# blyssprivacy/sdk

Hardware: NVIDIA H100
Metric: PIR server queries/sec (Spiral process_query) (higher is better)
Workload: dtype u64

## Files before the change

### sdk_b200/csrc/api.cu

```cuda
#include "api_internal.hpp"
#include "ntt_tables.hpp"
#include "update_body.hpp"
#include "gadget.hpp"
#include <cstdio>
#include <cerrno>
#include <fcntl.h>
#include <unistd.h>
#include <algorithm>
#include <cmath>
#include <memory>
#include <cstring>
#include <condition_variable>
#include <chrono>
#include <deque>
#include <mutex>
#include <set>
#include <utility>
#include <vector>

using namespace b200pir;

namespace b200pir {
thread_local unsigned long long g_kernel_launches = 0;
thread_local std::string g_last_error;

int fail(const std::exception& e) {
  cudaGetLastError();
  g_last_error = e.what();
  const Error* pe = dynamic_cast<const Error*>(&e);
  return pe ? pe->code : B200PIR_E_CUDA;
}

void opt_in_smem_impl(const void* kernel, int bytes) {
  static std::mutex mu;
  static std::set<std::pair<const void*, int>> done;
  int dev = 0;
  B200_CUDA(cudaGetDevice(&dev));
  std::lock_guard<std::mutex> lk(mu);
  if (done.count({kernel, dev})) return;
  B200_CUDA(cudaFuncSetAttribute(kernel, cudaFuncAttributeMaxDynamicSharedMemorySize, bytes));
  done.insert({kernel, dev});
}
}

namespace {

using b200pir::tables::build_tables;
using b200pir::tables::invmod;
uint64_t log2_ceil_u64(uint64_t a) { return (uint64_t)std::ceil(std::log2((double)a)); }
using b200pir::bits_per;
using b200pir::live_digits;
const uint64_t kQ2Values[37] = {0, 0, 0, 0, 0, 0, 0, 0, 0, 0, 0, 0, 0, 0, 12289ULL, 12289ULL, 61441ULL, 65537ULL,
                                65537ULL, 520193ULL, 786433ULL, 786433ULL, 3604481ULL, 7340033ULL, 16515073ULL,
                                33292289ULL, 67043329ULL, 132120577ULL, 268369921ULL, 469762049ULL, 1073479681ULL,
                                2013265921ULL, 4293918721ULL, 8588886017ULL, 17175674881ULL, 34359214081ULL,
                                68718428161ULL};

enum Stage { ST_EXPAND = 0, ST_MUL, ST_FROMNTT, ST_FOLD, ST_PACK, ST_ENCODE, ST_QIMG , ST_COUNT };

}

struct b200pir_ctx {
  int device = 0;
  cudaStream_t stream = nullptr;
  bool own_stream = true;
  std::recursive_mutex mu;
  b200pir_params hp;
  int dim0, num_per, slices, trials, g, stop_round, num_packing;
  int bits_gsw, bits_conv, bits_left, bits_right;
  int live_gsw, live_conv, live_left, live_right;
  bool has_right;
  uint64_t q2, q1, setup_bytes, query_bytes, response_bytes;
  int q1_bits;
  DevParams dp;
  DevBuf<Twiddle> d_tw;
  DevBuf<Twiddle> d_tw4k;
  DevBuf<uint32_t> d_neg1;
  int mul_variant = 0, max_group = 16, profile = 0;
  int sparse_fold = 0;
  int db_format = -1;
  DevBuf<uint2> w_qf;
  DevBuf<uint8_t> w_qt;
  int sm_count = 0;
  size_t ws_queries = 0, ws_rows = 0;
  DevBuf<uint64_t> w_query;
  DevBuf<uint32_t> w_v;
  DevBuf<uint32_t> w_zflags;
  DevBuf<uint32_t> w_xr;
  DevBuf<uint4> w_qdev;
  DevBuf<uint32_t> w_vfold, w_vfold_neg;
  DevBuf<uint32_t> w_mult;
  DevBuf<uint32_t> w_cts;
  const uint32_t* folded = nullptr;
  size_t folded_stride = 0;
  DevBuf<uint64_t> w_packed;
  DevBuf<uint8_t> w_resp;
  static constexpr size_t kWriteStageBytes = (size_t)64 << 20;
  static constexpr size_t kWriteStageItems = 65536;
  DevBuf<uint8_t> w_wbytes;
  DevBuf<ItemWrite> w_witems;
  std::mutex export_mu;
  uint8_t* h_export[2] = {nullptr, nullptr};
  size_t h_export_bytes = 0;
  cudaEvent_t export_done[2] = {nullptr, nullptr};
  void ensure_export_staging(size_t bytes) {
    w_wbytes.ensure(std::max(kWriteStageBytes, bytes));
    if (!export_done[0])
      for (auto& e : export_done) B200_CUDA(cudaEventCreateWithFlags(&e, cudaEventDisableTiming | cudaEventBlockingSync));
    if (bytes <= h_export_bytes) return;
    release_export_pinned();
    const size_t n = std::max(kWriteStageBytes, bytes);
    for (auto& h : h_export) B200_CUDA(cudaHostAlloc(reinterpret_cast<void**>(&h), n, cudaHostAllocDefault));
    h_export_bytes = n;
  }
  void release_export_pinned() {
    for (auto& h : h_export) { if (h) cudaFreeHost(h); h = nullptr; }
    h_export_bytes = 0;
  }
  struct Pending {
    b200pir_db* db; b200pir_pp* pp; const uint64_t* query_ct; const uint8_t* query_bytes; uint8_t* out;
    int rc = 0; std::string err; bool done = false;
  };
  static constexpr size_t kCoalesceMax = 32;
  static constexpr size_t kPassQueries = 16;
  int coalesce = 1;
  int coalesce_window_us = 200;
  size_t last_batch = 0;
  std::chrono::steady_clock::time_point last_batch_end{};
  std::mutex qmu;
  std::condition_variable qcv;
  std::deque<Pending*> pending;
  bool leader_active = false;
  unsigned long long coalesced_batches = 0, coalesced_queries = 0;
  DevBuf<const uint32_t*> d_pptab;
  size_t pptab_cap = 0;
  std::vector<const uint32_t*> h_pptab;
  b200pir_pp* const* multi_pps = nullptr;
  PpTable pp_table(b200pir_pp* pp, size_t count);
  struct Span { int stage; cudaEvent_t a, b; };
  std::vector<Span> spans;
  std::vector<cudaEvent_t> event_pool;
  size_t event_next = 0;
  int mul_launches = 0;
  double last_ms[9] = {0, 0, 0, 0, 0, 0, 0, 0, 0};

  size_t v_words() const { return ((size_t)1 << g) * 4 * POLY; }
  size_t fold_words() const { return (size_t)hp.nu_2 * 2 * 2 * hp.t_gsw * 2 * POLY; }
  MulGeom geom(int rows) const { return MulGeom{dim0, rows, slices}; }

  cudaEvent_t get_event() {
    if (event_next == event_pool.size()) {
      cudaEvent_t e;
      B200_CUDA(cudaEventCreate(&e));
      event_pool.push_back(e);
    }
    return event_pool[event_next++];
  }
  struct Scope {
    b200pir_ctx* c; int stage; cudaEvent_t a = nullptr;
    Scope(b200pir_ctx* ctx, int st) : c(ctx), stage(st) {
      if (c->profile) { a = c->get_event(); cudaEventRecord(a, c->stream); }
    }
    ~Scope() {
      if (c->profile) { cudaEvent_t b = c->get_event(); cudaEventRecord(b, c->stream); c->spans.push_back({stage, a, b}); }
    }
  };
  void prof_reset() { if (profile == 2) return; spans.clear(); event_next = 0; mul_launches = 0; }
  void prof_collect() {
    if (!profile) return;
    B200_CUDA(cudaStreamSynchronize(stream));
    for (int i = 0; i < 9; i++) last_ms[i] = 0;
    for (auto& s : spans) {
      float ms = 0;
      cudaEventElapsedTime(&ms, s.a, s.b);
      last_ms[s.stage == ST_QIMG ? 8 : s.stage] += ms;
      last_ms[6] += ms;
    }
    last_ms[7] = mul_launches;
  }
  void ensure_workspace_lite(size_t queries, size_t rows) {
    w_mult.ensure(queries * slices * rows * 4 * POLY);
    w_cts.ensure(queries * slices * rows * 4 * POLY);
    w_packed.ensure(queries * hp.instances * (hp.n + 1) * hp.n * POLY);
  }
  void ensure_workspace(size_t queries, size_t rows) {
    if (queries <= ws_queries && rows <= ws_rows) return;
    queries = std::max(queries, ws_queries);
    rows = std::max(rows, ws_rows);
    w_query.ensure(queries * 2 * POLY);
    if (hp.expand_queries) w_v.ensure(queries * v_words());
    w_qdev.ensure(queries * (size_t)dim0 * POLY);
    w_vfold.ensure(queries * std::max<size_t>(fold_words(), 1));
    w_vfold_neg.ensure(queries * std::max<size_t>(fold_words(), 1));
    w_mult.ensure(queries * slices * rows * 4 * POLY);
    w_cts.ensure(queries * slices * rows * 4 * POLY);
    w_packed.ensure(queries * hp.instances * (hp.n + 1) * hp.n * POLY);
    w_resp.ensure(queries * response_bytes);
    ws_queries = queries;
    ws_rows = rows;
  }
};

struct b200pir_db {
  b200pir_ctx* ctx;
  Shard shard;
  int rows;
  DbLayout layout;
  DevBuf<uint8_t> store;
  bool zmajor_product() const { return layout.format != 0; }
  uint4* slice0_base(int s, DevBuf<uint8_t>& scratch) {
    if (layout.format == 0) return reinterpret_cast<uint4*>(store.p);
    const size_t slice0_bytes = imad_cell(layout.G, 1, 0, 0, 0) * sizeof(uint4);
    if (!scratch.p) scratch.alloc(slice0_bytes);
    return reinterpret_cast<uint4*>(reinterpret_cast<uintptr_t>(scratch.p) - (uintptr_t)s * slice0_bytes);
  }
  void place_slice0(int s, const DevBuf<uint8_t>& scratch, cudaStream_t st) {
    const uint4* src = reinterpret_cast<const uint4*>(scratch.p);
    if (layout.format == 1) launch_db_to_frag(layout.F, src, reinterpret_cast<uint4*>(store.p), s, st);
    else if (layout.format == 2) launch_db_to_tc5(layout.T, src, store.p, s, st);
  }
  std::vector<uint64_t> present;
  uint64_t present_count = 0;
  std::vector<uint32_t> h_tile_mask;
  DevBuf<uint32_t> tile_mask;
  uint64_t capacity() const { return (uint64_t)ctx->slices * rows * ctx->dim0; }
  void presence_init() {
    present.assign((capacity() + 63) / 64, 0);
    present_count = 0;
    h_tile_mask.assign((size_t)ctx->slices * layout.T.mt, 0u);
    tile_mask.alloc(h_tile_mask.size());
    B200_CUDA(cudaMemsetAsync(tile_mask.p, 0, h_tile_mask.size() * 4, ctx->stream));
  }
  bool mark_host(int slice, int il, int j) {
    const uint64_t bit = ((uint64_t)slice * rows + il) * ctx->dim0 + j;
    if (!((present[bit >> 6] >> (bit & 63)) & 1)) { present[bit >> 6] |= 1ull << (bit & 63); present_count++; }
    const size_t w = (size_t)slice * layout.T.mt + (il >> 5);
    const uint32_t nv = h_tile_mask[w] | (1u << (j >> 5));
    if (nv == h_tile_mask[w]) return false;
    h_tile_mask[w] = nv;
    return true;
  }
  void mark(int slice, int il, int j, cudaStream_t s) {
    if (mark_host(slice, il, j)) {
      const size_t w = (size_t)slice * layout.T.mt + (il >> 5);
      B200_CUDA(cudaMemcpyAsync(tile_mask.p + w, &h_tile_mask[w], 4, cudaMemcpyHostToDevice, s));
    }
  }
  void mark_items(const ItemWrite* items, size_t count, cudaStream_t s) {
    bool changed = false;
    for (size_t k = 0; k < count; k++)
      for (int sl = 0; sl < ctx->slices; sl++) changed |= mark_host(sl, (int)items[k].il, (int)items[k].j);
    if (changed)
      B200_CUDA(cudaMemcpyAsync(tile_mask.p, h_tile_mask.data(), h_tile_mask.size() * 4, cudaMemcpyHostToDevice, s));
  }
  void mark_slice(int slice, cudaStream_t s) {
    const uint64_t lo = (uint64_t)slice * rows * ctx->dim0, hi = lo + (uint64_t)rows * ctx->dim0;
    for (uint64_t b = lo; b < hi; b++)
      if (!((present[b >> 6] >> (b & 63)) & 1)) { present[b >> 6] |= 1ull << (b & 63); present_count++; }
    const Tc5Geom& T = layout.T;
    const uint32_t full = T.ks >= 32 ? 0xffffffffu : ((1u << T.ks) - 1u);
    for (int m = 0; m < T.mt; m++) h_tile_mask[(size_t)slice * T.mt + m] = full;
    B200_CUDA(cudaMemcpyAsync(tile_mask.p + (size_t)slice * T.mt, &h_tile_mask[(size_t)slice * T.mt], (size_t)T.mt * 4,
                              cudaMemcpyHostToDevice, s));
  }
};

struct b200pir_pp {
  b200pir_ctx* ctx;
  DevBuf<uint32_t> pack, left, right, conv;
};

PpTable b200pir_ctx::pp_table(b200pir_pp* pp, size_t count) {
  if (count > pptab_cap) {
    pptab_cap = std::max<size_t>(count, 16);
    d_pptab.alloc(4 * pptab_cap);
    h_pptab.clear();
  }
  std::vector<const uint32_t*> h(4 * pptab_cap, nullptr);
  for (size_t i = 0; i < count; i++) {
    const b200pir_pp* p = multi_pps ? multi_pps[i] : pp;
    h[0 * pptab_cap + i] = p->pack.p;
    h[1 * pptab_cap + i] = p->left.p;
    h[2 * pptab_cap + i] = p->right.p ? p->right.p : p->left.p;
    h[3 * pptab_cap + i] = p->conv.p;
  }
  if (h != h_pptab) {
    B200_CUDA(cudaMemcpyAsync(d_pptab.p, h.data(), h.size() * sizeof(const uint32_t*), cudaMemcpyHostToDevice, stream));
    h_pptab = h;
  }
  return PpTable{d_pptab.p, d_pptab.p + pptab_cap, d_pptab.p + 2 * pptab_cap, d_pptab.p + 3 * pptab_cap};
}

namespace {

struct Guard {
  std::lock_guard<std::recursive_mutex> lk;
  explicit Guard(b200pir_ctx* c) : lk(c->mu) { cudaSetDevice(c->device); }
};

void upload_narrow(b200pir_ctx* c, uint32_t* dst, DevBuf<uint64_t>& wide, const uint64_t* host, size_t words) {
  wide.ensure(words);
  B200_CUDA(cudaMemcpyAsync(wide.p, host, words * 8, cudaMemcpyHostToDevice, c->stream));
  launch_narrow(dst, wide.p, words, c->stream);
}
void download_widen(b200pir_ctx* c, uint64_t* host, const uint32_t* src, size_t words) {
  DevBuf<uint64_t> wide(words);
  launch_widen(wide.p, src, words, c->stream);
  B200_CUDA(cudaMemcpyAsync(host, wide.p, words * 8, cudaMemcpyDeviceToHost, c->stream));
  B200_CUDA(cudaStreamSynchronize(c->stream));
}
void upload_ntt32(b200pir_ctx* c, DevBuf<uint32_t>& dst, const uint64_t* host, size_t words) {
  dst.alloc(words);
  DevBuf<uint64_t> wide;
  upload_narrow(c, dst.p, wide, host, words);
  B200_CUDA(cudaStreamSynchronize(c->stream));
}


void run_coefficient_expansion(b200pir_ctx* c, b200pir_pp* pp, uint32_t* v, size_t v_stride, int nq, bool all_slots) {
  const auto& hp = c->hp;
  cudaStream_t s = c->stream;
  const int g = c->g;
  const int stop_round = hp.nu_2 > 0 ? c->stop_round : 0;
  const int max_right = hp.nu_2 > 0 ? (int)(hp.t_gsw * hp.nu_2) : 0;
  const PpTable T = c->pp_table(pp, (size_t)nq);
  for (int r = 0; r < g; r++) {
    const int num_in = 1 << r;
    ExpandRound R;
    R.r = r; R.num_in = num_in; R.stop_round = stop_round; R.max_bits_to_gen_right = max_right;
    R.fill_skipped = all_slots ? 1 : 0;
    R.t_auto = (POLY >> r) + 1;
    R.t_left = (int)hp.t_exp_left; R.bits_left = c->bits_left; R.live_left = c->live_left;
    R.tab_left = T.left; R.off_left = (size_t)r * 2 * hp.t_exp_left * 2 * POLY;
    if (hp.nu_2 > 0 && c->has_right) {
      int rr = r <= c->stop_round ? r : c->stop_round;
      R.t_right = (int)hp.t_exp_right; R.bits_right = c->bits_right; R.live_right = c->live_right;
      R.tab_right = T.right; R.off_right = (size_t)rr * 2 * hp.t_exp_right * 2 * POLY;
    } else {
      R.t_right = R.t_left; R.bits_right = R.bits_left; R.live_right = R.live_left; R.tab_right = T.left; R.off_right = R.off_left;
    }
    const size_t xr_stride = (size_t)num_in * 2 * POLY;
    c->w_xr.ensure((size_t)nq * xr_stride);
    launch_expand_round_res(c->dp, v, v_stride, c->w_xr.p, xr_stride, nq, R, c->d_neg1.p + (size_t)r * 2 * POLY, s);
  }
}

void run_expand_query(b200pir_ctx* c, b200pir_pp* pp, const uint64_t* query_raw, uint32_t* v, uint4* q_dev,
                      uint32_t* v_fold, int nq, uint8_t* images = nullptr) {
  const auto& hp = c->hp;
  cudaStream_t s = c->stream;
  launch_to_ntt_strided(c->dp, v, c->v_words(), query_raw, (size_t)2 * POLY, 2, nq, s);
  run_coefficient_expansion(c, pp, v, c->v_words(), nq, false);
  const int factor = hp.nu_2 > 0 ? 2 : 1;
  if (images) {
    const Tc5Geom T = make_tc5_geom(c->dim0, 32);
    for (int q0 = 0; q0 < nq; q0 += 16)
      launch_reorient_to_tc5(T, v + (size_t)q0 * c->v_words(), c->v_words(), factor, std::min(16, nq - q0),
                             images + (size_t)(q0 / 16) * tc5_query_bytes(T), s);
  } else {
    launch_reorient(c->geom(c->num_per), q_dev, (size_t)c->dim0 * POLY, v, c->v_words(), nq, factor, s);
  }
  if (hp.nu_2 > 0)
    launch_regev_to_gsw(c->dp, v_fold, c->fold_words(), v, c->v_words(), nq, (int)hp.nu_2, 2, 1, c->pp_table(pp, (size_t)nq).conv,
                        (int)hp.t_gsw, (int)hp.t_conv, c->bits_conv, c->live_conv, s);
}

void run_fold(b200pir_ctx* c, uint64_t* cts, size_t batch, size_t batch_stride, size_t num, int k0,
              const uint32_t* vfold, const uint32_t* vfold_neg, int slices_per_query) {
  const size_t mat = (size_t)2 * 2 * c->hp.t_gsw * 2 * POLY;
  int k = k0;
  for (size_t half = num / 2; half >= 1; half /= 2, k--) {
    launch_fold_round(c->dp, cts, batch, batch_stride, (int)half, vfold + (size_t)k * mat, vfold_neg + (size_t)k * mat,
                      c->fold_words(), slices_per_query, (int)c->hp.t_gsw, c->bits_gsw, c->stream);
  }
}

const uint32_t* run_fold_res(b200pir_ctx* c, uint32_t* a, uint32_t* b, size_t batch, size_t batch_stride, size_t num,
                             int k0, const uint32_t* vfold, int slices_per_query) {
  const size_t mat = (size_t)2 * 2 * c->hp.t_gsw * 2 * POLY;
  int k = k0;
  uint32_t* src = a;
  uint32_t* dst = b;
  uint32_t* zero_flags = nullptr;
  if (c->sparse_fold) {
    c->w_zflags.ensure(batch * num);
    zero_flags = c->w_zflags.p;
  }
  for (size_t half = num / 2; half >= 1; half /= 2, k--) {
    launch_fold_res(c->dp, src, dst, batch, batch_stride, (int)half, vfold + (size_t)k * mat, c->fold_words(),
                    slices_per_query, (int)c->hp.t_gsw, c->bits_gsw, c->live_gsw, zero_flags, c->stream);
    std::swap(src, dst);
  }
  return src;
}

void run_prepare(b200pir_ctx* c, b200pir_pp* pp, size_t count, bool images = false) {
  b200pir_ctx::Scope sc(c, ST_EXPAND);
  if (images) c->w_qt.ensure((count + 15) / 16 * tc5_query_bytes(make_tc5_geom(c->dim0, 32)));
  if (c->hp.expand_queries)
    run_expand_query(c, pp, c->w_query.p, c->w_v.p, c->w_qdev.p, c->w_vfold.p, (int)count, images ? c->w_qt.p : nullptr);
}

void run_first_dim(b200pir_ctx* c, b200pir_db* db, size_t count, const uint4* qdev, uint32_t* out, int slice_begin,
                   int slice_count, const uint8_t* images = nullptr, size_t per_group = 16) {
  const DbLayout& L = db->layout;
  const size_t q_stride = (size_t)c->dim0 * POLY;
  const size_t out_stride = (size_t)c->slices * db->rows * 4 * POLY;
  if (L.format == 0) {
    b200pir_ctx::Scope sc(c, ST_MUL);
    size_t qi = 0;
    while (qi < count) {
      int nq = 1;
      if (count - qi >= 4 && c->max_group >= 4) nq = 4;
      else if (count - qi >= 2 && c->max_group >= 2) nq = 2;
      launch_multiply(c->dp, L.G, reinterpret_cast<const uint4*>(L.base), qdev + qi * q_stride, out + qi * out_stride,
                      slice_begin, slice_count, nq, q_stride, out_stride, c->mul_variant, c->stream);
      c->mul_launches++;
      qi += nq;
    }
  } else if (L.format == 2) {
    if (!images) c->w_qt.ensure(tc5_query_bytes(L.T));
    const size_t step = images ? per_group : 16;
    for (size_t qi = 0, g = 0; qi < count; qi += step, g++) {
      const int nq = (int)std::min<size_t>(step, count - qi);
      const uint8_t* qt = images ? images + g * tc5_query_bytes(L.T) : c->w_qt.p;
      if (!images) {
        b200pir_ctx::Scope sq(c, ST_QIMG);
        launch_query_to_tc5(L.T, qdev + qi * q_stride, q_stride, nq, c->w_qt.p, c->stream);
      }
      b200pir_ctx::Scope sc(c, ST_MUL);
      launch_multiply_tc5(c->dp, L.T, L.base, db->tile_mask.p, qt, out + qi * out_stride, out_stride, nq, slice_begin,
                          slice_count, c->sm_count, c->stream);
      c->mul_launches++;
    }
  } else {
    c->w_qf.ensure(imma_query_cells(L.F));
    const size_t per_pass = (c->max_group >= 16 && imma_supports_16(L.F)) ? 16 : (c->max_group >= 8 ? 8 : 4);
    for (size_t qi = 0; qi < count; qi += per_pass) {
      const int nq = (int)std::min<size_t>(per_pass, count - qi);
      {
        b200pir_ctx::Scope sq(c, ST_QIMG);
        launch_query_to_frag(L.F, qdev + qi * q_stride, q_stride, nq, c->w_qf.p, c->stream);
      }
      {
        b200pir_ctx::Scope sc(c, ST_MUL);
        launch_multiply_imma(c->dp, L.F, reinterpret_cast<const uint4*>(L.base), c->w_qf.p, out + qi * out_stride, out_stride,
                             nq, slice_begin, slice_count, c->stream);
        c->mul_launches++;
      }
    }
  }
}

void run_first_dim_and_fold(b200pir_ctx* c, b200pir_db* db, size_t count, const uint4* qdev = nullptr,
                            const uint32_t* vfold = nullptr, const uint8_t* images = nullptr, size_t per_group = 16) {
  if (!qdev) qdev = c->w_qdev.p;
  if (!vfold) vfold = c->w_vfold.p;
  const int rows = db->rows;
  const size_t out_stride = (size_t)c->slices * rows * 4 * POLY;
  const bool zmajor = db->zmajor_product();
  run_first_dim(c, db, count, qdev, zmajor ? c->w_cts.p : c->w_mult.p, 0, c->slices, images, per_group);
  {
    b200pir_ctx::Scope sc(c, ST_FROMNTT);
    if (zmajor) launch_intt_from_zmajor(c->dp, db->layout.F, c->w_cts.p, out_stride, c->w_mult.p, (int)count, c->slices, c->stream);
    else launch_ntt32(c->dp, c->w_mult.p, count * c->slices * rows * 2, true, c->stream);
  }
  {
    b200pir_ctx::Scope sc(c, ST_FOLD);
    c->folded = c->w_mult.p;
    c->folded_stride = (size_t)rows * 4 * POLY;
    if (rows > 1)
      c->folded = run_fold_res(c, c->w_mult.p, c->w_cts.p, count * c->slices, (size_t)rows * 4 * POLY, rows,
                               (int)c->hp.nu_2 - 1, vfold, c->slices);
  }
}

void run_pack_encode(b200pir_ctx* c, b200pir_pp* pp, const uint32_t* folded, size_t ct_stride, size_t count,
                     uint8_t* out_dev) {
  const auto& hp = c->hp;
  const size_t packed_words = (size_t)hp.instances * (hp.n + 1) * hp.n * POLY;
  {
    b200pir_ctx::Scope sc(c, ST_PACK);
    launch_pack(c->dp, c->w_packed.p, packed_words, folded, ct_stride, (size_t)c->slices * ct_stride, (int)count, c->pp_table(pp, count).pack,
                (int)hp.n, (int)hp.instances, (int)hp.t_conv, c->bits_conv, c->live_conv, (int)hp.version, c->stream);
  }
  {
    b200pir_ctx::Scope sc(c, ST_ENCODE);
    launch_encode(c->dp, out_dev, c->response_bytes, c->w_packed.p, packed_words, (int)count, (int)hp.n, (int)hp.instances,
                  c->q2, (int)hp.q2_bits, c->q1, c->q1_bits, c->stream);
  }
}

bool same_params(const b200pir_ctx* a, const b200pir_ctx* b) {
  return a == b || (a->device == b->device && std::memcmp(&a->hp, &b->hp, sizeof(b200pir_params)) == 0);
}
void check_db(b200pir_ctx* c, b200pir_db* db) {
  if (!db || !same_params(db->ctx, c)) throw Error(B200PIR_E_BADARG, "db handle was created for different parameters / device");
}
void check_pp(b200pir_ctx* c, b200pir_pp* pp) {
  if (!pp || !same_params(pp->ctx, c)) throw Error(B200PIR_E_BADARG, "pp handle was created for different parameters / device");
}

}

extern "C" {

const char* b200pir_last_error(void) { return g_last_error.c_str(); }
int b200pir_device_count(void) {
  int n = 0;
  if (cudaGetDeviceCount(&n) != cudaSuccess) return 0;
  return n;
}

int b200pir_ctx_create(const b200pir_params* params, int device, b200pir_ctx** out) {
  API_BEGIN
  if (!params || !out) throw Error(B200PIR_E_BADARG, "null argument");
  use_device(device);
  std::unique_ptr<b200pir_ctx> c(new b200pir_ctx());
  c->device = device;
  B200_CUDA(cudaDeviceGetAttribute(&c->sm_count, cudaDevAttrMultiProcessorCount, device));
  c->hp = *params;
  auto& hp = c->hp;
  if (hp.q2_bits < 14) hp.q2_bits = 14;
  if (hp.q2_bits > 36) throw Error(B200PIR_E_BADARG, "q2_bits out of range");
  if (hp.instances == 0) hp.instances = 1;
  if (hp.n < 1 || hp.n > 4) throw Error(B200PIR_E_UNSUPPORTED, "n must be 1..4");
  if (hp.nu_1 < 1 || hp.nu_1 > 16 || hp.nu_2 > 16) throw Error(B200PIR_E_BADARG, "nu_1/nu_2 out of range");
  if (hp.version > 1) throw Error(B200PIR_E_BADARG, "unknown version");
  if (hp.p < 2 || (hp.p & (hp.p - 1)) || hp.p > (1u << 20)) throw Error(B200PIR_E_BADARG, "p must be a power of two <= 2^20");
  for (uint64_t t : {hp.t_gsw, hp.t_conv, hp.t_exp_left, hp.t_exp_right})
    if (t < 3 || t > 56)
      throw Error(B200PIR_E_UNSUPPORTED, "gadget dimensions must be in 3..56");
  if (hp.db_item_size == 0) hp.db_item_size = hp.instances * hp.n * hp.n * 2048 * log2_ceil_u64(hp.p) / 8;
  c->dim0 = 1 << hp.nu_1;
  c->num_per = 1 << hp.nu_2;
  c->trials = (int)(hp.n * hp.n);
  c->slices = (int)(hp.instances * c->trials);
  c->g = (int)log2_ceil_u64(hp.t_gsw * hp.nu_2 + c->dim0);
  c->stop_round = hp.nu_2 ? (int)log2_ceil_u64(hp.t_gsw * hp.nu_2) : 0;
  if (c->g > 11) throw Error(B200PIR_E_UNSUPPORTED, "expansion needs more than 2048 slots");
  if (hp.expand_queries && hp.nu_2 > 0 && 2 * std::max<uint64_t>(c->dim0, hp.t_gsw * hp.nu_2) > (1ull << c->g))
    throw Error(B200PIR_E_UNSUPPORTED, "expansion: dim0 and t_gsw * nu_2 must each fit in half of the 2^g slots");
  c->num_packing = hp.version == 0 ? (int)hp.n : 2;
  c->has_right = hp.expand_queries && (hp.version == 0 || hp.t_exp_right != hp.t_exp_left);
  c->bits_gsw = bits_per((int)hp.t_gsw);
  c->bits_conv = bits_per((int)hp.t_conv);
  c->bits_left = bits_per((int)hp.t_exp_left);
  c->bits_right = bits_per((int)hp.t_exp_right);
  c->live_gsw = live_digits((int)hp.t_gsw);
  c->live_conv = live_digits((int)hp.t_conv);
  c->live_left = live_digits((int)hp.t_exp_left);
  c->live_right = live_digits((int)hp.t_exp_right);
  c->q2 = kQ2Values[hp.q2_bits];
  c->q1 = 4 * hp.p;
  c->q1_bits = (int)log2_ceil_u64(c->q1);
  {
    uint64_t bits = hp.instances * (hp.q2_bits * hp.n * 2048 + (uint64_t)c->q1_bits * hp.n * hp.n * 2048);
    c->response_bytes = ((bits + 63) / 64) * 8;
    uint64_t sz = (uint64_t)c->num_packing * hp.n * hp.t_conv;
    if (hp.expand_queries) {
      uint64_t right = (uint64_t)(c->stop_round + 1) * hp.t_exp_right;
      if (hp.version > 0 && hp.t_exp_left == hp.t_exp_right) right = 0;
      sz += (uint64_t)c->g * hp.t_exp_left + right + 2 * hp.t_conv;
    }
    c->setup_bytes = 32 + sz * 2048 * 8;
    uint64_t qp = hp.expand_queries ? 1 : (uint64_t)c->dim0 + hp.nu_2 * 2 * hp.t_gsw;
    c->query_bytes = 32 + qp * 2048 * 8;
  }
  B200_CUDA(cudaStreamCreateWithFlags(&c->stream, cudaStreamNonBlocking));
  const uint64_t q0 = 268369921ULL, q1m = 249561089ULL;
  std::vector<Twiddle> f0, i0, f1, i1;
  build_tables(q0, f0, i0);
  build_tables(q1m, f1, i1);
  std::vector<Twiddle> l0, l1;
  b200pir::tables::build_inverse_table_lz(q0, l0);
  b200pir::tables::build_inverse_table_lz(q1m, l1);
  c->d_tw.alloc(6 * POLY);
  const size_t tw_bytes = POLY * sizeof(Twiddle);
  B200_CUDA(cudaMemcpyAsync(c->d_tw.p + 4 * POLY, l0.data(), tw_bytes, cudaMemcpyHostToDevice, c->stream));
  B200_CUDA(cudaMemcpyAsync(c->d_tw.p + 5 * POLY, l1.data(), tw_bytes, cudaMemcpyHostToDevice, c->stream));
  B200_CUDA(cudaMemcpyAsync(c->d_tw.p, f0.data(), tw_bytes, cudaMemcpyHostToDevice, c->stream));
  B200_CUDA(cudaMemcpyAsync(c->d_tw.p + POLY, i0.data(), tw_bytes, cudaMemcpyHostToDevice, c->stream));
  B200_CUDA(cudaMemcpyAsync(c->d_tw.p + 2 * POLY, f1.data(), tw_bytes, cudaMemcpyHostToDevice, c->stream));
  B200_CUDA(cudaMemcpyAsync(c->d_tw.p + 3 * POLY, i1.data(), tw_bytes, cudaMemcpyHostToDevice, c->stream));
  std::vector<Twiddle> lo(2 * 3 * 64);
  for (int i = 0; i < 64; i++) { lo[(0 * 3 + 0) * 64 + i] = f0[i]; lo[(0 * 3 + 1) * 64 + i] = i0[i]; lo[(0 * 3 + 2) * 64 + i] = l0[i];
                                 lo[(1 * 3 + 0) * 64 + i] = f1[i]; lo[(1 * 3 + 1) * 64 + i] = i1[i]; lo[(1 * 3 + 2) * 64 + i] = l1[i]; }
  upload_poly_constants(lo.data(), c->stream);
  upload_mul_constants(lo.data(), c->stream);
  upload_imma_constants(lo.data(), c->stream);
  std::vector<Twiddle> tw4k;
  for (const uint64_t q : {q0, q1m}) {
    std::vector<Twiddle> f, i;
    build_tables(q, f, i, 4096, 12);
    tw4k.insert(tw4k.end(), f.begin(), f.end());
    tw4k.insert(tw4k.end(), i.begin(), i.end());
  }
  c->d_tw4k.alloc(tw4k.size());
  B200_CUDA(cudaMemcpyAsync(c->d_tw4k.p, tw4k.data(), tw4k.size() * sizeof(Twiddle), cudaMemcpyHostToDevice, c->stream));
  DevParams& dp = c->dp;
  dp.q[0] = (uint32_t)q0; dp.q[1] = (uint32_t)q1m;
  dp.cr1[0] = (uint64_t)(((u128)1 << 64) / q0);
  dp.cr1[1] = (uint64_t)(((u128)1 << 64) / q1m);
  dp.modulus = q0 * q1m;
  dp.cr1_mod = (uint64_t)(((u128)1 << 64) / dp.modulus);
  dp.q1_inv_mod_q0 = (uint32_t)invmod(q1m % q0, q0);
  dp.fwd[0] = c->d_tw.p; dp.inv[0] = c->d_tw.p + POLY; dp.fwd[1] = c->d_tw.p + 2 * POLY; dp.inv[1] = c->d_tw.p + 3 * POLY;
  dp.inv_lz[0] = c->d_tw.p + 4 * POLY; dp.inv_lz[1] = c->d_tw.p + 5 * POLY;
  dp.mu58[0] = (uint32_t)(((uint64_t)1 << 58) / q0); dp.mu58[1] = (uint32_t)(((uint64_t)1 << 58) / q1m);
  {
    std::vector<uint32_t> h((size_t)NTT_LOG_N * 2 * POLY, 0);
    for (int i = 0; i < NTT_LOG_N; i++) {
      int idx = POLY - (1 << i);
      h[((size_t)i * 2 + 0) * POLY + idx] = (uint32_t)(q0 - 1);
      h[((size_t)i * 2 + 1) * POLY + idx] = (uint32_t)(q1m - 1);
    }
    c->d_neg1.alloc(h.size());
    B200_CUDA(cudaMemcpyAsync(c->d_neg1.p, h.data(), h.size() * 4, cudaMemcpyHostToDevice, c->stream));
    launch_ntt32(dp, c->d_neg1.p, NTT_LOG_N, false, c->stream);
    B200_CUDA(cudaStreamSynchronize(c->stream));
  }
  B200_CUDA(cudaGetLastError());
  *out = c.release();
  API_END
}

void b200pir_ctx_destroy(b200pir_ctx* c) {
  if (!c) return;
  cudaSetDevice(c->device);
  cudaDeviceSynchronize();
  for (auto e : c->event_pool) cudaEventDestroy(e);
  c->release_export_pinned();
  for (auto e : c->export_done) if (e) cudaEventDestroy(e);
  if (c->own_stream && c->stream) cudaStreamDestroy(c->stream);
  delete c;
}
int b200pir_ctx_set_stream(b200pir_ctx* c, void* cuda_stream) {
  API_BEGIN
  if (!c) throw Error(B200PIR_E_BADARG, "null ctx");
  Guard gd(c);
  B200_CUDA(cudaStreamSynchronize(c->stream));
  if (c->own_stream && c->stream) cudaStreamDestroy(c->stream);
  c->stream = (cudaStream_t)cuda_stream;
  c->own_stream = false;
  API_END
}
int b200pir_ctx_synchronize(b200pir_ctx* c) {
  API_BEGIN
  if (!c) throw Error(B200PIR_E_BADARG, "null ctx");
  Guard gd(c);
  B200_CUDA(cudaStreamSynchronize(c->stream));
  B200_CUDA(cudaGetLastError());
  API_END
}
int b200pir_ctx_reserve(b200pir_ctx* c, size_t queries, size_t rows_local) {
  API_BEGIN
  if (!c) throw Error(B200PIR_E_BADARG, "null ctx");
  if (queries == 0 || queries > 4096 || rows_local == 0 || rows_local > ((size_t)1 << c->hp.nu_2))
    throw Error(B200PIR_E_BADARG, "reserve: 1..4096 queries, 1..num_per rows");
  Guard gd(c);
  B200_CUDA(cudaStreamSynchronize(c->stream));
  c->ensure_workspace(queries, rows_local);
  B200_CUDA(cudaGetLastError());
  API_END
}
int b200pir_ctx_set_option(b200pir_ctx* c, const char* key, int64_t value) {
  API_BEGIN
  if (!c || !key) throw Error(B200PIR_E_BADARG, "null argument");
  Guard gd(c);
  std::string k(key);
  if (k == "mul_variant") c->mul_variant = (int)value;
  else if (k == "batch") { if (value != 1 && value != 2 && value != 4 && value != 8 && value != 16) throw Error(B200PIR_E_BADARG, "batch must be 1, 2, 4, 8 or 16"); c->max_group = (int)value; }
  else if (k == "fold_variant" || k == "intt_variant" || k == "imma_variant" || k == "expand_variant" ||
           k == "expand_pair_min_ctas") {}
  else if (k == "sparse_fold") c->sparse_fold = value != 0;
  else if (k == "coalesce") c->coalesce = value != 0;
  else if (k == "coalesce_window_us") { if (value < 0 || value > 100000) throw Error(B200PIR_E_BADARG, "coalesce_window_us must be 0..100000"); c->coalesce_window_us = (int)value; }
  else if (k == "db_format") { if (value < -1 || value > 2) throw Error(B200PIR_E_BADARG, "db_format must be -1 (automatic), 0, 1 or 2"); c->db_format = (int)value; }
  else if (k == "profile") {
    if (value < 0 || value > 2) throw Error(B200PIR_E_BADARG, "profile must be 0, 1 or 2");
    c->profile = (int)value;
    c->spans.clear(); c->event_next = 0; c->mul_launches = 0;
  }
  else throw Error(B200PIR_E_BADARG, "unknown option " + k);
  API_END
}
int b200pir_ctx_sizes(b200pir_ctx* c, uint64_t* setup_bytes, uint64_t* query_bytes, uint64_t* response_bytes) {
  API_BEGIN
  if (!c) throw Error(B200PIR_E_BADARG, "null ctx");
  if (setup_bytes) *setup_bytes = c->setup_bytes;
  if (query_bytes) *query_bytes = c->query_bytes;
  if (response_bytes) *response_bytes = c->response_bytes;
  API_END
}

int b200pir_db_create(b200pir_ctx* c, uint64_t shard_index, uint64_t shard_count, b200pir_db** out) {
  API_BEGIN
  if (!c || !out) throw Error(B200PIR_E_BADARG, "null argument");
  Guard gd(c);
  if (shard_count == 0) { shard_count = 1; shard_index = 0; }
  if (shard_index >= shard_count || (shard_count & (shard_count - 1)) || (uint64_t)c->num_per % shard_count)
    throw Error(B200PIR_E_BADARG, "shard_count must be a power of two dividing num_per");
  std::unique_ptr<b200pir_db> db(new b200pir_db());
  db->ctx = c;
  db->shard = Shard{(int)shard_index, (int)shard_count};
  db->rows = c->num_per / (int)shard_count;
  DbLayout& L = db->layout;
  L.G = c->geom(db->rows);
  L.F = make_imma_geom(c->dim0, db->rows);
  L.T = make_tc5_geom(c->dim0, db->rows);
  L.format = c->db_format >= 0 ? c->db_format : (tc5_supported(L.T) ? 2 : 1);
  db->presence_init();
  if (L.format == 2 && !tc5_supported(L.T)) throw Error(B200PIR_E_UNSUPPORTED, "db_format 2: dim0 too large for the wgmma kernel");
  db->store.alloc(db_bytes(L, c->slices));
  L.base = db->store.p;
  B200_CUDA(cudaMemsetAsync(db->store.p, 0, db->store.n, c->stream));
  B200_CUDA(cudaStreamSynchronize(c->stream));
  *out = db.release();
  API_END
}
void b200pir_db_destroy(b200pir_db* db) {
  if (!db) return;
  cudaSetDevice(db->ctx->device);
  delete db;
}
extern "C++" {
namespace {
template <typename Fetch>
void upload_slice_impl(b200pir_ctx* c, b200pir_db* db, uint64_t slice, Fetch fetch) {
  const size_t per_z = (size_t)c->dim0 * c->num_per;
  int zc = (int)std::max<size_t>(1, std::min<size_t>(POLY, ((size_t)64 << 20) / (per_z * 8)));
  DevBuf<uint64_t> stage(per_z * zc);
  const MulGeom& G = db->layout.G;
  DevBuf<uint8_t> scratch;
  uint4* dst = db->slice0_base((int)slice, scratch) + imad_cell(G, (int)slice, 0, 0, 0);
  for (int z0 = 0; z0 < POLY; z0 += zc) {
    int cur = std::min(zc, POLY - z0);
    const uint64_t* src = fetch((size_t)z0 * per_z, per_z * cur);
    B200_CUDA(cudaMemcpyAsync(stage.p, src, per_z * cur * 8, cudaMemcpyHostToDevice, c->stream));
    launch_db_retile_chunk(G, db->shard, dst, stage.p, z0, cur, c->stream);
    B200_CUDA(cudaStreamSynchronize(c->stream));
  }
  db->place_slice0((int)slice, scratch, c->stream);
  db->mark_slice((int)slice, c->stream);
  B200_CUDA(cudaStreamSynchronize(c->stream));
  B200_CUDA(cudaGetLastError());
}

void write_items(b200pir_ctx* c, b200pir_db* db, const uint8_t* host, size_t span, const ItemWrite* items, size_t count) {
  if (count == 0) return;
  c->w_wbytes.ensure(std::max(b200pir_ctx::kWriteStageBytes, span));
  c->w_witems.ensure(std::max(b200pir_ctx::kWriteStageItems, count));
  if (span) B200_CUDA(cudaMemcpyAsync(c->w_wbytes.p, host, span, cudaMemcpyHostToDevice, c->stream));
  B200_CUDA(cudaMemcpyAsync(c->w_witems.p, items, count * sizeof(ItemWrite), cudaMemcpyHostToDevice, c->stream));
  const size_t chunks = (size_t)c->slices;
  const size_t bpc = (c->hp.db_item_size + chunks - 1) / chunks;
  launch_write_items(c->dp, db->layout, c->w_wbytes.p, c->w_witems.p, (int)count, (int)chunks, (int)bpc, c->hp.p, c->stream);
}

template <typename Sink>
void export_impl(b200pir_ctx* c, b200pir_db* db, int slice_begin, int slice_end, Sink sink) {
  std::lock_guard<std::mutex> ex(c->export_mu);
  const size_t per_z = (size_t)db->rows * c->dim0;
  const int zc = (int)std::max<size_t>(1, std::min<size_t>(POLY, b200pir_ctx::kWriteStageBytes / (per_z * 8)));
  struct Chunk { int slice, z0, zc; };
  std::vector<Chunk> chunks;
  for (int s = slice_begin; s < slice_end; s++)
    for (int z0 = 0; z0 < POLY; z0 += zc) chunks.push_back(Chunk{s, z0, std::min(zc, POLY - z0)});
  {
    Guard gd(c);
    c->ensure_export_staging(per_z * zc * 8);
  }
  auto consume = [&](size_t k) {
    const int b = (int)(k & 1);
    B200_CUDA(cudaEventSynchronize(c->export_done[b]));
    sink(chunks[k].slice, chunks[k].z0, chunks[k].zc, reinterpret_cast<const uint64_t*>(c->h_export[b]));
  };
  try {
    for (size_t k = 0; k < chunks.size(); k++) {
      {
        Guard gd(c);
        uint64_t* stage = reinterpret_cast<uint64_t*>(c->w_wbytes.p);
        launch_db_export(db->layout, chunks[k].slice, chunks[k].z0, chunks[k].zc, stage, c->stream);
        B200_CUDA(cudaMemcpyAsync(c->h_export[k & 1], stage, per_z * chunks[k].zc * 8, cudaMemcpyDeviceToHost, c->stream));
        B200_CUDA(cudaEventRecord(c->export_done[k & 1], c->stream));
      }
      if (k > 0) consume(k - 1);
    }
    if (!chunks.empty()) consume(chunks.size() - 1);
  } catch (...) {
    for (auto e : c->export_done) cudaEventSynchronize(e);
    throw;
  }
  B200_CUDA(cudaGetLastError());
}

void download_impl(b200pir_ctx* c, b200pir_db* db, int slice_begin, int slice_end, uint64_t* words) {
  const size_t d0 = (size_t)c->dim0, npg = (size_t)c->num_per, rows = (size_t)db->rows;
  const size_t G = (size_t)db->shard.count, gi = (size_t)db->shard.index;
  const size_t slice_words = d0 * npg * POLY;
  export_impl(c, db, slice_begin, slice_end, [&](int s, int z0, int zc, const uint64_t* src) {
    uint64_t* dst = words + (size_t)(s - slice_begin) * slice_words + (size_t)z0 * npg * d0;
    if (G == 1) { std::memcpy(dst, src, (size_t)zc * rows * d0 * 8); return; }
    for (size_t zl = 0; zl < (size_t)zc; zl++)
      for (size_t il = 0; il < rows; il++)
        std::memcpy(dst + (zl * npg + il * G + gi) * d0, src + (zl * rows + il) * d0, d0 * 8);
  });
}
}
}

int b200pir_db_upload_slice(b200pir_ctx* c, b200pir_db* db, uint64_t slice, const uint64_t* words, size_t n_words) {
  API_BEGIN
  if (!c || !words) throw Error(B200PIR_E_BADARG, "null argument");
  Guard gd(c);
  check_db(c, db);
  const size_t slice_words = (size_t)c->dim0 * c->num_per * POLY;
  if (slice >= (uint64_t)c->slices) throw Error(B200PIR_E_SHAPE, "slice out of range");
  if (n_words != slice_words) throw Error(B200PIR_E_SHAPE, "slice must hold dim0*num_per*2048 words");
  upload_slice_impl(c, db, slice, [&](size_t off, size_t) { return words + off; });
  API_END
}
int b200pir_db_load_file(b200pir_ctx* c, b200pir_db* db, const char* path) {
  API_BEGIN
  if (!c || !path) throw Error(B200PIR_E_BADARG, "null argument");
  Guard gd(c);
  check_db(c, db);
  const size_t slice_words = (size_t)c->dim0 * c->num_per * POLY;
// ... 453 lines not shown
  while (((size_t)1 << dims) < num) dims++;
  if (dims > (int)c->hp.nu_2) throw Error(B200PIR_E_SHAPE, "more ciphertexts than 2^nu_2");
  const size_t mat = (size_t)2 * 2 * c->hp.t_gsw * 2 * POLY;
  DevBuf<uint64_t> cts(num * 2 * POLY), wide;
  DevBuf<uint32_t> vf(c->fold_words());
  B200_CUDA(cudaMemcpyAsync(cts.p, v_cts, cts.n * 8, cudaMemcpyHostToDevice, c->stream));
  upload_narrow(c, vf.p, wide, v_folding, dims * mat);
  const bool has_q = std::find(v_cts, v_cts + cts.n, c->dp.modulus) != v_cts + cts.n;
  if ((v_folding_neg || has_q) && !c->sparse_fold) {
    DevBuf<uint32_t> vfn(c->fold_words());
    if (v_folding_neg) upload_narrow(c, vfn.p, wide, v_folding_neg, dims * mat);
    else launch_folding_neg(c->dp, vfn.p, vf.p, dims, (int)c->hp.t_gsw, c->bits_gsw, c->stream);
    run_fold(c, cts.p, 1, num * 2 * POLY, num, dims - 1, vf.p, vfn.p, 1);
  } else {
    DevBuf<uint32_t> a(num * 4 * POLY), b(num * 4 * POLY);
    DevBuf<uint32_t> zflags;
    if (c->sparse_fold) zflags.alloc(num);
    launch_raw_to_res(c->dp, a.p, cts.p, num * 2, c->stream);
    int k = dims - 1;
    for (size_t half = num / 2; half >= 1; half /= 2, k--) {
      launch_fold_res(c->dp, a.p, b.p, 1, num * 4 * POLY, (int)half, vf.p + (size_t)k * mat, c->fold_words(), 1,
                      (int)c->hp.t_gsw, c->bits_gsw, c->live_gsw, zflags.p, c->stream);
      B200_CUDA(cudaMemcpyAsync(a.p, b.p, half * 4 * POLY * 4, cudaMemcpyDeviceToDevice, c->stream));
    }
    launch_res_to_raw(c->dp, cts.p, a.p, num * 2, c->stream);
  }
  B200_CUDA(cudaMemcpyAsync(v_cts, cts.p, cts.n * 8, cudaMemcpyDeviceToHost, c->stream));
  B200_CUDA(cudaStreamSynchronize(c->stream));
  B200_CUDA(cudaGetLastError());
  API_END
}

int b200pir_get_v_folding_neg(b200pir_ctx* c, uint64_t* out, const uint64_t* v_folding) {
  API_BEGIN
  if (!c || !out || !v_folding) throw Error(B200PIR_E_BADARG, "null argument");
  Guard gd(c);
  const size_t words = c->fold_words();
  if (!words) return 0;
  DevBuf<uint64_t> wide;
  DevBuf<uint32_t> in(words), o(words);
  upload_narrow(c, in.p, wide, v_folding, words);
  launch_folding_neg(c->dp, o.p, in.p, (int)c->hp.nu_2, (int)c->hp.t_gsw, c->bits_gsw, c->stream);
  download_widen(c, out, o.p, words);
  B200_CUDA(cudaGetLastError());
  API_END
}

int b200pir_coefficient_expansion(b200pir_ctx* c, b200pir_pp* pp, uint64_t* v) {
  API_BEGIN
  if (!c || !v) throw Error(B200PIR_E_BADARG, "null argument");
  Guard gd(c);
  check_pp(c, pp);
  if (!c->hp.expand_queries) throw Error(B200PIR_E_BADARG, "context was created with expand_queries = 0");
  const size_t words = c->v_words();
  DevBuf<uint64_t> wide;
  DevBuf<uint32_t> dv(words);
  upload_narrow(c, dv.p, wide, v, words);
  run_coefficient_expansion(c, pp, dv.p, words, 1, true);
  download_widen(c, v, dv.p, words);
  B200_CUDA(cudaGetLastError());
  API_END
}

int b200pir_expand_query(b200pir_ctx* c, b200pir_pp* pp, const uint64_t* query_ct, uint64_t* out_v_firstdim,
                         uint64_t* out_v_folding) {
  API_BEGIN
  if (!c || !query_ct || !out_v_firstdim) throw Error(B200PIR_E_BADARG, "null argument");
  Guard gd(c);
  check_pp(c, pp);
  if (!c->hp.expand_queries) throw Error(B200PIR_E_BADARG, "context was created with expand_queries = 0");
  c->ensure_workspace(1, 1);
  B200_CUDA(cudaMemcpyAsync(c->w_query.p, query_ct, 2 * POLY * 8, cudaMemcpyHostToDevice, c->stream));
  run_expand_query(c, pp, c->w_query.p, c->w_v.p, c->w_qdev.p, c->w_vfold.p, 1);
  const size_t qwords = (size_t)c->dim0 * 2 * POLY;
  std::vector<uint32_t> hq(qwords * 2);
  B200_CUDA(cudaMemcpyAsync(hq.data(), c->w_qdev.p, hq.size() * 4, cudaMemcpyDeviceToHost, c->stream));
  B200_CUDA(cudaStreamSynchronize(c->stream));
  for (int j = 0; j < c->dim0; j++)
    for (int z = 0; z < POLY; z++) {
      const uint32_t* cell = hq.data() + (((size_t)(j >> 1) * 2 + (j & 1)) * POLY + z) * 4;
      out_v_firstdim[((size_t)z * c->dim0 + j) * 2 + 0] = (uint64_t)cell[0] | ((uint64_t)cell[1] << 32);
      out_v_firstdim[((size_t)z * c->dim0 + j) * 2 + 1] = (uint64_t)cell[2] | ((uint64_t)cell[3] << 32);
    }
  if (out_v_folding && c->fold_words()) download_widen(c, out_v_folding, c->w_vfold.p, c->fold_words());
  B200_CUDA(cudaGetLastError());
  API_END
}

int b200pir_pack(b200pir_ctx* c, b200pir_pp* pp, const uint64_t* v_ct, uint64_t* out_ntt) {
  API_BEGIN
  if (!c || !v_ct || !out_ntt) throw Error(B200PIR_E_BADARG, "null argument");
  Guard gd(c);
  check_pp(c, pp);
  const auto& hp = c->hp;
  const size_t nn = hp.n * hp.n, outp = (hp.n + 1) * hp.n;
  DevBuf<uint64_t> cts(nn * 2 * POLY), raw(outp * POLY);
  DevBuf<uint32_t> o(outp * 2 * POLY), res(nn * 4 * POLY);
  B200_CUDA(cudaMemcpyAsync(cts.p, v_ct, cts.n * 8, cudaMemcpyHostToDevice, c->stream));
  launch_raw_to_res(c->dp, res.p, cts.p, nn * 2, c->stream);
  launch_pack(c->dp, raw.p, 0, res.p, 4 * POLY, 0, 1, c->pp_table(pp, 1).pack, (int)hp.n, 1, (int)hp.t_conv, c->bits_conv, c->live_conv, (int)hp.version, c->stream,
              cts.p);
  launch_to_ntt(c->dp, o.p, raw.p, outp, c->stream);
  download_widen(c, out_ntt, o.p, o.n);
  B200_CUDA(cudaGetLastError());
  API_END
}

int b200pir_encode(b200pir_ctx* c, const uint64_t* v_packed_raw, uint8_t* out, size_t* out_len) {
  API_BEGIN
  if (!c || !v_packed_raw || !out) throw Error(B200PIR_E_BADARG, "null argument");
  Guard gd(c);
  const auto& hp = c->hp;
  const size_t words = (size_t)hp.instances * (hp.n + 1) * hp.n * POLY;
  DevBuf<uint64_t> in(words);
  DevBuf<uint8_t> o(c->response_bytes);
  B200_CUDA(cudaMemcpyAsync(in.p, v_packed_raw, words * 8, cudaMemcpyHostToDevice, c->stream));
  launch_encode(c->dp, o.p, c->response_bytes, in.p, 0, 1, (int)hp.n, (int)hp.instances, c->q2, (int)hp.q2_bits, c->q1, c->q1_bits, c->stream);
  B200_CUDA(cudaMemcpyAsync(out, o.p, c->response_bytes, cudaMemcpyDeviceToHost, c->stream));
  B200_CUDA(cudaStreamSynchronize(c->stream));
  if (out_len) *out_len = c->response_bytes;
  B200_CUDA(cudaGetLastError());
  API_END
}

extern "C++" {
namespace {
struct Responses {
  uint8_t* dev = nullptr;
  uint8_t* host = nullptr;
  uint8_t* const* each = nullptr;
  size_t* len = nullptr;
};

template <typename Stage>
void run_queries(b200pir_ctx* c, b200pir_db* db, b200pir_pp* pp, b200pir_pp* const* pps, size_t count, bool needs_expand,
                 Stage stage, const Responses& out) {
  Guard gd(c);
  check_db(c, db);
  if (pps)
    for (size_t i = 0; i < count; i++) check_pp(c, pps[i]);
  else
    check_pp(c, pp);
  if (db->shard.count != 1) throw Error(B200PIR_E_BADARG, "sharded database: use the stage_a / stage_b entry points");
  if (needs_expand && !c->hp.expand_queries)
    throw Error(B200PIR_E_BADARG, pps ? "multi-client batches need expand_queries" : "batch entry point needs expand_queries");
  if (count == 0) return;
  c->ensure_workspace(pps && c->coalesce ? std::max(count, b200pir_ctx::kCoalesceMax) : count, db->rows);
  c->prof_reset();
  stage();
  const bool images = db->layout.format == 2 && c->hp.expand_queries;
  if (pps) pp = pps[0];
  c->multi_pps = pps;
  try {
    run_prepare(c, pp, count, images);
    run_first_dim_and_fold(c, db, count, nullptr, nullptr, images ? c->w_qt.p : nullptr, 16);
    run_pack_encode(c, pp, c->folded, c->folded_stride, count, out.dev ? out.dev : c->w_resp.p);
  } catch (...) { c->multi_pps = nullptr; throw; }
  c->multi_pps = nullptr;
  if (!out.dev) {
    const size_t rb = c->response_bytes;
    if (out.each)
      for (size_t i = 0; i < count; i++)
        B200_CUDA(cudaMemcpyAsync(out.each[i], c->w_resp.p + i * rb, rb, cudaMemcpyDeviceToHost, c->stream));
    else
      B200_CUDA(cudaMemcpyAsync(out.host, c->w_resp.p, count * rb, cudaMemcpyDeviceToHost, c->stream));
    B200_CUDA(cudaStreamSynchronize(c->stream));
    if (c->profile == 1) c->prof_collect();
    if (out.len) *out.len = rb;
  }
  B200_CUDA(cudaGetLastError());
}

void stage_each(b200pir_ctx* c, const uint64_t* const* cts, const uint8_t* const* bytes, size_t count) {
  for (size_t i = 0; i < count; i++) {
    if (bytes && bytes[i]) deserialize_queries(c, bytes[i], 1, c->w_query.p + i * 2 * POLY);
    else B200_CUDA(cudaMemcpyAsync(c->w_query.p + i * 2 * POLY, cts[i], 2 * POLY * 8, cudaMemcpyHostToDevice, c->stream));
  }
}
}
}

int b200pir_process_query_batch_dev(b200pir_ctx* c, b200pir_db* db, b200pir_pp* pp, const uint64_t* query_cts_dev,
                                    size_t count, uint8_t* out_dev) {
  API_BEGIN
  if (!c || !out_dev || !query_cts_dev) throw Error(B200PIR_E_BADARG, "null argument");
  run_queries(c, db, pp, nullptr, count, true, [&] {
    B200_CUDA(cudaMemcpyAsync(c->w_query.p, query_cts_dev, count * 2 * POLY * 8, cudaMemcpyDeviceToDevice, c->stream));
  }, Responses{out_dev});
  API_END
}

int b200pir_process_query_batch(b200pir_ctx* c, b200pir_db* db, b200pir_pp* pp, const uint64_t* query_cts, size_t count,
                                uint8_t* out, size_t* out_len_each) {
  API_BEGIN
  if (!c || !out || !query_cts) throw Error(B200PIR_E_BADARG, "null argument");
  run_queries(c, db, pp, nullptr, count, true, [&] {
    B200_CUDA(cudaMemcpyAsync(c->w_query.p, query_cts, count * 2 * POLY * 8, cudaMemcpyHostToDevice, c->stream));
  }, Responses{nullptr, out, nullptr, out_len_each});
  API_END
}

namespace {
int coalesced_query(b200pir_ctx* c, b200pir_db* db, b200pir_pp* pp, const uint64_t* query_ct, const uint8_t* query_bytes,
                    uint8_t* out) {
  b200pir_ctx::Pending me;
  me.db = db; me.pp = pp; me.query_ct = query_ct; me.query_bytes = query_bytes; me.out = out;
  std::unique_lock<std::mutex> lk(c->qmu);
  c->pending.push_back(&me);
  c->qcv.notify_all();
  while (!me.done) {
    if (c->leader_active) { c->qcv.wait(lk); continue; }
    c->leader_active = true;
    if (c->coalesce_window_us > 0 && c->last_batch > 1 && c->pending.size() < std::min(c->last_batch, b200pir_ctx::kPassQueries)) {
      const auto now = std::chrono::steady_clock::now();
      if (now - c->last_batch_end < std::chrono::milliseconds(1)) {
        const size_t want = std::min(c->last_batch, b200pir_ctx::kPassQueries);
        c->qcv.wait_until(lk, now + std::chrono::microseconds(c->coalesce_window_us), [&] { return c->pending.size() >= want; });
      }
    }
    std::vector<b200pir_ctx::Pending*> batch;
    b200pir_db* bdb = c->pending.front()->db;
    size_t avail = 0;
    for (auto* p : c->pending) avail += p->db == bdb;
    size_t take = std::min(avail, b200pir_ctx::kCoalesceMax);
    if (take > b200pir_ctx::kPassQueries) take -= take % b200pir_ctx::kPassQueries;
    for (auto it = c->pending.begin(); it != c->pending.end() && batch.size() < take;) {
      if ((*it)->db == bdb) { batch.push_back(*it); it = c->pending.erase(it); } else ++it;
    }
    lk.unlock();
    int rc = 0;
    std::string err;
    try {
      std::vector<b200pir_pp*> pps; std::vector<const uint64_t*> cts; std::vector<const uint8_t*> bys; std::vector<uint8_t*> outs;
      for (auto* p : batch) { pps.push_back(p->pp); cts.push_back(p->query_ct); bys.push_back(p->query_bytes); outs.push_back(p->out); }
      run_queries(c, bdb, nullptr, pps.data(), batch.size(), true, [&] { stage_each(c, cts.data(), bys.data(), batch.size()); },
                  Responses{nullptr, nullptr, outs.data()});
    } catch (const std::exception& e) { rc = fail(e); err = e.what(); }
    lk.lock();
    c->coalesced_batches++; c->coalesced_queries += batch.size();
    c->last_batch = batch.size();
    c->last_batch_end = std::chrono::steady_clock::now();
    for (auto* p : batch) { p->rc = rc; p->err = err; p->done = true; }
    c->leader_active = false;
    c->qcv.notify_all();
  }
  if (me.rc) g_last_error = me.err;
  return me.rc;
}
}

int b200pir_process_queries(b200pir_ctx* c, b200pir_db* db, b200pir_pp* const* pps, const uint64_t* const* query_cts, size_t count,
                            uint8_t* const* outs) {
  API_BEGIN
  if (!c || !pps || !query_cts || !outs) throw Error(B200PIR_E_BADARG, "null argument");
  for (size_t i = 0; i < count; i++)
    if (!pps[i] || !query_cts[i] || !outs[i]) throw Error(B200PIR_E_BADARG, "null entry");
  if (count == 0) return 0;
  run_queries(c, db, nullptr, pps, count, true, [&] { stage_each(c, query_cts, nullptr, count); }, Responses{nullptr, nullptr, outs});
  API_END
}
int b200pir_coalesce_stats(b200pir_ctx* c, uint64_t* batches, uint64_t* queries) {
  API_BEGIN
  if (!c) throw Error(B200PIR_E_BADARG, "null ctx");
  std::lock_guard<std::mutex> lk(c->qmu);
  if (batches) *batches = c->coalesced_batches;
  if (queries) *queries = c->coalesced_queries;
  API_END
}

int b200pir_process_query_bytes(b200pir_ctx* c, b200pir_db* db, b200pir_pp* pp, const uint8_t* queries, size_t len,
                                size_t count, uint8_t* out, size_t* out_len_each) {
  API_BEGIN
  if (!c || !out || !queries) throw Error(B200PIR_E_BADARG, "null argument");
  if (len != count * c->query_bytes) throw Error(B200PIR_E_SHAPE, "queries: expected " + std::to_string(count * c->query_bytes) + " bytes");
  if (count == 1 && c->coalesce && c->hp.expand_queries && db && pp) {
    const int rc = coalesced_query(c, db, pp, nullptr, queries, out);
    if (rc == 0 && out_len_each) *out_len_each = c->response_bytes;
    return rc;
  }
  run_queries(c, db, pp, nullptr, count, false, [&] {
    if (c->hp.expand_queries) {
      deserialize_queries(c, queries, count, c->w_query.p);
    } else {
      for (size_t i = 0; i < count; i++) deserialize_query_direct(c, queries + i * c->query_bytes, i);
    }
  }, Responses{nullptr, out, nullptr, out_len_each});
  API_END
}

int b200pir_process_query(b200pir_ctx* c, b200pir_db* db, b200pir_pp* pp, const uint64_t* query_ct, const uint64_t* v_buf,
                          const uint64_t* v_ct, uint8_t* out, size_t* out_len) {
  if (!c) { g_last_error = "null ctx"; return B200PIR_E_BADARG; }
  if (c->hp.expand_queries) {
    if (!query_ct || !out || !db || !pp) { g_last_error = "null argument"; return B200PIR_E_BADARG; }
    if (!c->coalesce) return b200pir_process_query_batch(c, db, pp, query_ct, 1, out, out_len);
    const int rc = coalesced_query(c, db, pp, query_ct, nullptr, out);
    if (rc == 0 && out_len) *out_len = c->response_bytes;
    return rc;
  }
  API_BEGIN
  if (!v_buf || (!v_ct && c->hp.nu_2) || !out) throw Error(B200PIR_E_BADARG, "null argument");
  DevBuf<uint64_t> vq, raw;
  run_queries(c, db, pp, nullptr, 1, false, [&] {
    vq.alloc((size_t)c->dim0 * 2 * POLY);
    B200_CUDA(cudaMemcpyAsync(vq.p, v_buf, vq.n * 8, cudaMemcpyHostToDevice, c->stream));
    launch_query_to_dev(c->geom(db->rows), c->w_qdev.p, vq.p, c->stream);
    const size_t npolys = (size_t)c->hp.nu_2 * 2 * 2 * c->hp.t_gsw;
    raw.alloc(std::max<size_t>(npolys, 1) * POLY);
// ... 199 lines not shown
```

Measured before the change: 1568.

## Overlap regev-to-GSW conversion with first-dimension multiply on a side stream

```diff
diff --git a/sdk_b200/csrc/api.cu b/sdk_b200/csrc/api.cu
--- a/sdk_b200/csrc/api.cu
+++ b/sdk_b200/csrc/api.cu
@@ -82,6 +82,10 @@
   DevBuf<uint2> w_qf;
   DevBuf<uint8_t> w_qt;
   int sm_count = 0;
+  static constexpr int kMulCtas = 128;
+  int mul_ctas = kMulCtas;
+  cudaStream_t side = nullptr;
+  cudaEvent_t conv_ready = nullptr, conv_done = nullptr;
   size_t ws_queries = 0, ws_rows = 0;
   DevBuf<uint64_t> w_query;
   DevBuf<uint32_t> w_v;
@@ -346,7 +350,7 @@
 }
 
 void run_expand_query(b200pir_ctx* c, b200pir_pp* pp, const uint64_t* query_raw, uint32_t* v, uint4* q_dev,
-                      uint32_t* v_fold, int nq, uint8_t* images = nullptr) {
+                      uint32_t* v_fold, int nq, uint8_t* images = nullptr, cudaStream_t conv_stream = nullptr) {
   const auto& hp = c->hp;
   cudaStream_t s = c->stream;
   launch_to_ntt_strided(c->dp, v, c->v_words(), query_raw, (size_t)2 * POLY, 2, nq, s);
@@ -360,9 +364,16 @@
   } else {
     launch_reorient(c->geom(c->num_per), q_dev, (size_t)c->dim0 * POLY, v, c->v_words(), nq, factor, s);
   }
-  if (hp.nu_2 > 0)
-    launch_regev_to_gsw(c->dp, v_fold, c->fold_words(), v, c->v_words(), nq, (int)hp.nu_2, 2, 1, c->pp_table(pp, (size_t)nq).conv,
-                        (int)hp.t_gsw, (int)hp.t_conv, c->bits_conv, c->live_conv, s);
+  if (hp.nu_2 > 0) {
+    const uint32_t* const* conv = c->pp_table(pp, (size_t)nq).conv;
+    if (conv_stream) {
+      B200_CUDA(cudaEventRecord(c->conv_ready, s));
+      B200_CUDA(cudaStreamWaitEvent(conv_stream, c->conv_ready, 0));
+    }
+    launch_regev_to_gsw(c->dp, v_fold, c->fold_words(), v, c->v_words(), nq, (int)hp.nu_2, 2, 1, conv, (int)hp.t_gsw,
+                        (int)hp.t_conv, c->bits_conv, c->live_conv, conv_stream ? conv_stream : s);
+    if (conv_stream) B200_CUDA(cudaEventRecord(c->conv_done, conv_stream));
+  }
 }
 
 void run_fold(b200pir_ctx* c, uint64_t* cts, size_t batch, size_t batch_stride, size_t num, int k0,
@@ -394,15 +405,16 @@
   return src;
 }
 
-void run_prepare(b200pir_ctx* c, b200pir_pp* pp, size_t count, bool images = false) {
+void run_prepare(b200pir_ctx* c, b200pir_pp* pp, size_t count, bool images = false, cudaStream_t conv_stream = nullptr) {
   b200pir_ctx::Scope sc(c, ST_EXPAND);
   if (images) c->w_qt.ensure((count + 15) / 16 * tc5_query_bytes(make_tc5_geom(c->dim0, 32)));
   if (c->hp.expand_queries)
-    run_expand_query(c, pp, c->w_query.p, c->w_v.p, c->w_qdev.p, c->w_vfold.p, (int)count, images ? c->w_qt.p : nullptr);
+    run_expand_query(c, pp, c->w_query.p, c->w_v.p, c->w_qdev.p, c->w_vfold.p, (int)count, images ? c->w_qt.p : nullptr,
+                     conv_stream);
 }
 
 void run_first_dim(b200pir_ctx* c, b200pir_db* db, size_t count, const uint4* qdev, uint32_t* out, int slice_begin,
-                   int slice_count, const uint8_t* images = nullptr, size_t per_group = 16) {
+                   int slice_count, const uint8_t* images = nullptr, size_t per_group = 16, int sms = 0) {
   const DbLayout& L = db->layout;
   const size_t q_stride = (size_t)c->dim0 * POLY;
   const size_t out_stride = (size_t)c->slices * db->rows * 4 * POLY;
@@ -430,7 +442,7 @@
       }
       b200pir_ctx::Scope sc(c, ST_MUL);
       launch_multiply_tc5(c->dp, L.T, L.base, db->tile_mask.p, qt, out + qi * out_stride, out_stride, nq, slice_begin,
-                          slice_count, c->sm_count, c->stream);
+                          slice_count, sms > 0 ? sms : c->sm_count, c->stream);
       c->mul_launches++;
     }
   } else {
@@ -453,13 +465,16 @@
 }
 
 void run_first_dim_and_fold(b200pir_ctx* c, b200pir_db* db, size_t count, const uint4* qdev = nullptr,
-                            const uint32_t* vfold = nullptr, const uint8_t* images = nullptr, size_t per_group = 16) {
+                            const uint32_t* vfold = nullptr, const uint8_t* images = nullptr, size_t per_group = 16,
+                            bool conv_beside = false) {
   if (!qdev) qdev = c->w_qdev.p;
   if (!vfold) vfold = c->w_vfold.p;
   const int rows = db->rows;
   const size_t out_stride = (size_t)c->slices * rows * 4 * POLY;
   const bool zmajor = db->zmajor_product();
-  run_first_dim(c, db, count, qdev, zmajor ? c->w_cts.p : c->w_mult.p, 0, c->slices, images, per_group);
+  run_first_dim(c, db, count, qdev, zmajor ? c->w_cts.p : c->w_mult.p, 0, c->slices, images, per_group,
+                conv_beside ? c->mul_ctas : 0);
+  if (conv_beside) B200_CUDA(cudaStreamWaitEvent(c->stream, c->conv_done, 0));
   {
     b200pir_ctx::Scope sc(c, ST_FROMNTT);
     if (zmajor) launch_intt_from_zmajor(c->dp, db->layout.F, c->w_cts.p, out_stride, c->w_mult.p, (int)count, c->slices, c->stream);
@@ -568,6 +583,13 @@
     c->query_bytes = 32 + qp * 2048 * 8;
   }
   B200_CUDA(cudaStreamCreateWithFlags(&c->stream, cudaStreamNonBlocking));
+  {
+    int least = 0, greatest = 0;
+    B200_CUDA(cudaDeviceGetStreamPriorityRange(&least, &greatest));
+    B200_CUDA(cudaStreamCreateWithPriority(&c->side, cudaStreamNonBlocking, least));
+    B200_CUDA(cudaEventCreateWithFlags(&c->conv_ready, cudaEventDisableTiming));
+    B200_CUDA(cudaEventCreateWithFlags(&c->conv_done, cudaEventDisableTiming));
+  }
   const uint64_t q0 = 268369921ULL, q1m = 249561089ULL;
   std::vector<Twiddle> f0, i0, f1, i1;
   build_tables(q0, f0, i0);
@@ -630,6 +652,8 @@
   cudaSetDevice(c->device);
   cudaDeviceSynchronize();
   for (auto e : c->event_pool) cudaEventDestroy(e);
+  for (auto e : {c->conv_ready, c->conv_done}) if (e) cudaEventDestroy(e);
+  if (c->side) cudaStreamDestroy(c->side);
   c->release_export_pinned();
   for (auto e : c->export_done) if (e) cudaEventDestroy(e);
   if (c->own_stream && c->stream) cudaStreamDestroy(c->stream);
@@ -674,6 +698,10 @@
   else if (k == "fold_variant" || k == "intt_variant" || k == "imma_variant" || k == "expand_variant" ||
            k == "expand_pair_min_ctas") {}
   else if (k == "sparse_fold") c->sparse_fold = value != 0;
+  else if (k == "mul_ctas") {
+    if (value < 0 || value > c->sm_count) throw Error(B200PIR_E_BADARG, "mul_ctas must be 0..the device's SM count");
+    c->mul_ctas = (int)value;
+  }
   else if (k == "coalesce") c->coalesce = value != 0;
   else if (k == "coalesce_window_us") { if (value < 0 || value > 100000) throw Error(B200PIR_E_BADARG, "coalesce_window_us must be 0..100000"); c->coalesce_window_us = (int)value; }
   else if (k == "db_format") { if (value < -1 || value > 2) throw Error(B200PIR_E_BADARG, "db_format must be -1 (automatic), 0, 1 or 2"); c->db_format = (int)value; }
@@ -1433,8 +1461,9 @@
   if (pps) pp = pps[0];
   c->multi_pps = pps;
   try {
-    run_prepare(c, pp, count, images);
-    run_first_dim_and_fold(c, db, count, nullptr, nullptr, images ? c->w_qt.p : nullptr, 16);
+    const bool conv_beside = images && c->mul_ctas > 0 && !c->profile && c->hp.nu_2 > 0;
+    run_prepare(c, pp, count, images, conv_beside ? c->side : nullptr);
+    run_first_dim_and_fold(c, db, count, nullptr, nullptr, images ? c->w_qt.p : nullptr, 16, conv_beside);
     run_pack_encode(c, pp, c->folded, c->folded_stride, count, out.dev ? out.dev : c->w_resp.p);
   } catch (...) { c->multi_pps = nullptr; throw; }
   c->multi_pps = nullptr;
```

Result: faster. 1586 (median of 6 runs) (+1.2%).
